# ReactiveBayes/RxInfer.jl

Hardware: AMD Instinct MI355X
Metric: node-message-updates/sec (d=4 LGSSM, T=100k, BP sweep with Bethe free energy) (higher is better)
Workload: dtype f64; 1 GPU; LGSSM d=4 dy=4 T=100000, 1024 independent chains per GPU (BASELINE config 2), 1 BP sweep + Bethe free energy per step; chain c drawn from numpy default_rng(42+c); chains_per_gpu=1024, T=100000, segments=128, segment_len=782

## Files before the change

### rxinfer.jl_amd/csrc/lgssm_kernels.hpp

```cpp
#pragma once
#include <hip/hip_runtime.h>
#include <stdint.h>

namespace rxhip {

constexpr int ST_NOT_POSDEF = 1;
constexpr int ST_NONFINITE = 2;
__device__ __forceinline__ void lds_barrier() {
    __builtin_amdgcn_fence(__ATOMIC_RELEASE, "workgroup", "local");
    __builtin_amdgcn_s_barrier();
    __builtin_amdgcn_fence(__ATOMIC_ACQUIRE, "workgroup", "local");
}
__device__ __forceinline__ bool is_finite(double x) { return (__double2hiint(x) & 0x7ff00000) != 0x7ff00000; }

#ifndef RXHIP_NT_STORES
#define RXHIP_NT_STORES 0
#endif
typedef double rx_d2v __attribute__((ext_vector_type(2)));
__device__ __forceinline__ void stream_store(double2* p, double a, double b) {
#if RXHIP_NT_STORES
    rx_d2v v = {a, b};
    __builtin_nontemporal_store(v, reinterpret_cast<rx_d2v*>(p));
#else
    *p = make_double2(a, b);
#endif
}

template <int D>
struct Dim {
    static constexpr int NS = D * (D + 1) / 2;
    static constexpr int NP = D + NS;
    static constexpr int NP2 = (NP + 1) / 2;
};

__host__ __device__ constexpr int sidx(int i, int j) { return i >= j ? i * (i + 1) / 2 + j : j * (j + 1) / 2 + i; }
// ... 965 lines not shown
    for (int q = 0; q < NS; ++q) {
        al[AL::J + q] = x[(EX::J + q) * p.n_chains];
        al[AL::C + q] = x[(EX::C + q) * p.n_chains];
    }
    if (!derived) return true;
    Sym<D> C, Ci;
    double det;
#pragma unroll
    for (int q = 0; q < NS; ++q) C.v[q] = al[AL::C + q];
    const bool ok = spd_inv<D>(C, Ci, det);
#pragma unroll
    for (int q = 0; q < NS; ++q) al[AL::CI + q] = Ci.v[q];
#pragma unroll
    for (int a = 0; a < D; ++a)
#pragma unroll
        for (int c = 0; c < D; ++c) {
            double acc = 0.0;
#pragma unroll
            for (int k = 0; k < D; ++k) acc += Ci(a, k) * al[AL::PI + k * D + c];
            al[AL::X + a * D + c] = acc;
        }
#pragma unroll
    for (int a = 0; a < D; ++a)
#pragma unroll
        for (int c = 0; c <= a; ++c) {
            double acc = al[AL::J + sidx(a, c)];
#pragma unroll
            for (int k = 0; k < D; ++k) acc += al[AL::PI + k * D + a] * al[AL::X + k * D + c];
            al[AL::JJ + sidx(a, c)] = acc;
        }
    return ok;
}

template <int D, int DY, bool FE, bool CK = false>
__global__ void __launch_bounds__(64) k_forward0(Params p, const CstArg<CstLayout<D, DY>::SIZE> cb) {
    using CL = CstLayout<D, DY>;
    using FL = F0Layout<D, DY>;
    constexpr int MT = TimeTab<D>::MT;
    constexpr int MP2 = DimM<D>::MP2;
    constexpr int U = 4;
    constexpr int NPF = U * FL::SIZE / 2;
    constexpr int NPM = U * MT / 2;
    constexpr int NPC = NPF + NPM;
    constexpr int PPL = (NPC + 63) / 64;
    __shared__ double2 tbuf[2][NPC];
    const int lane = threadIdx.x;
    const long long g = (long long)blockIdx.x * blockDim.x + threadIdx.x;
    const long long total = p.n_chains * (long long)p.S;
    const bool live = g < total;
    const long long seg = live ? g / p.n_chains : 0;
    const long long chain = live ? g - seg * p.n_chains : 0;
    const long long len = live ? seg_len(p, seg) : 0;
    const CPtr c{cb.v};
    const long long t0 = seg * p.L + 1;
    const long long seg0 = __builtin_amdgcn_readfirstlane((int)seg);
    const bool straddle = __builtin_amdgcn_ballot_w64(live && seg != seg0) != 0;
    const long long tw0 = seg0 * p.L + 1;
    const long long f_pieces = p.L * (FL::SIZE / 2);
    const long long m_pieces = p.T * (MT / 2);
    const double2* f2 = reinterpret_cast<const double2*>(p.ftab);
    const double2* m2 = reinterpret_cast<const double2*>(p.mtab);

    double2 tr[PPL];
    auto fetch = [&](long long i0) {
#pragma unroll
        for (int k = 0; k < PPL; ++k) {
// ... 2120 lines not shown
    constexpr int NS = Dim<D>::NS;
    {
        double mp[D], yv[DY];
        Sym<D> Vp, V;
#pragma unroll
        for (int i = 0; i < D; ++i) mp[i] = c[CL::M1 + i];
#pragma unroll
        for (int i = 0; i < NS; ++i) Vp.v[i] = c[CL::V1 + i];
        load_y<DY>(p.y, 0, p.n_chains, chain, yv);
        bool ok = true;
        double quad = 0.0, detprod = 1.0;
        obs_update<D, DY, true>(c, mp, Vp, yv, mseg, V, ok, quad, detprod);
        if (seg == 0) {
            store_filt_sh<D>(p, 0, chain, mseg, V);
            if (fe) p.fe_part[chain] = -0.5 * (quad + log(detprod));
            if (!ok) atomicOr(p.status, ST_NOT_POSDEF);
        }
    }
    boundary_chain<D, false>(p, chain - lane, (unsigned)lane, 0, (int)seg, lds, mseg);
#pragma unroll
    for (int i = 0; i < D; ++i) xb[i] = 0.0;
    boundary_chain<D, true>(p, chain - lane, (unsigned)lane, p.S - 1, p.S - 1 - (int)seg, lds, xb);
    const double* row = p.scan + seg * SL::SIZE;
    Sym<D> Vb, Lb;
#pragma unroll
    for (int i = 0; i < NS; ++i) {
        Vb.v[i] = row[SL::VB + i];
        Lb.v[i] = (seg == p.S - 1) ? 0.0 : row[SL::LB + i];
    }
    store_soa<D>(p.fstart, seg, p.n_chains, chain, mseg, Vb);
    store_soa<D>(p.beta, seg + 1, p.n_chains, chain, xb, Lb);
}

template <int D, int DY>
__global__ void __launch_bounds__(64) k_backward_sh_rev(Params p, const double* __restrict__ gtab, const double* __restrict__ segend,
                                                        const CstArg<CstLayout<D, DY>::SIZE> cb, const int bnd, const int write_cov) {
    using ST = SmoothTab<D>;
    using CL = CstLayout<D, DY>;
    constexpr int MP2 = DimM<D>::MP2;
    constexpr int MT = TimeTab<D>::MT;
    constexpr int U = 4;
    constexpr int RP = ST::SIZE / 2;
    constexpr int NPC = U * RP;
    constexpr int PPL = (NPC + 63) / 64;
    constexpr int NMP = 32 * D;
    constexpr int NCP = 32 * D * D;
    __shared__ double2 tbuf[2][NPC];
    __shared__ double mtile[64 * D];
    __shared__ double bndbuf[2][BndStage<D>::N];
    const int lane = threadIdx.x;
    const long long g0 = (long long)blockIdx.x * 64;
    const long long seg = g0 / p.n_chains;
    const long long chain0 = g0 - seg * p.n_chains;
    const long long chain = chain0 + lane;
    const long long len = seg_len(p, seg);
    const long long tb = seg * p.L, te = tb + len;
    const CPtr c{cb.v};
    const int lg = p.ck_log2;
    const long long K = 1LL << lg;
    auto load_ck = [&](long long t, double2 (&r)[MP2]) { load_filt_m_sh<D>(p, 1 + seg * p.nck + ((t - tb - 1) >> lg), chain, r); };
    double mseg[D];
    auto ck_mean = [&](const double2 (&r)[MP2], long long t, double (&mf)[D]) {
        unpack_m_sh<D>(r, mf);
        const double* N = p.ntab + t * MT;
#pragma unroll
        for (int i = 0; i < D; ++i) {
            double s = mf[i];
#pragma unroll
            for (int k = 0; k < D; ++k) s += N[i * D + k] * mseg[k];
            mf[i] = s;
        }
    };

    double mf[D], ms[D];
    {
        double xb[D];
        if (bnd) boundary_in_sweep<D, DY>(p, c, seg, chain, lane, bnd == 2, bndbuf, mseg, xb);
        else {
            const double* q = p.fstart + (seg * Dim<D>::NP) * p.n_chains + chain;
            const double* bq = p.beta + ((seg + 1) * Dim<D>::NP) * p.n_chains + chain;
#pragma unroll
            for (int i = 0; i < D; ++i) {
                mseg[i] = q[i * p.n_chains];
                xb[i] = bq[i * p.n_chains];
            }
        }
        if (len > 0) {
            double2 r[MP2];
            load_ck(te, r);
            ck_mean(r, te, mf);
        } else {
#pragma unroll
            for (int i = 0; i < D; ++i) mf[i] = mseg[i];
        }
        const double* se = segend + seg * SegEndTab<D>::SIZE;
#pragma unroll
        for (int i = 0; i < D; ++i) {
            double s = 0.0;
#pragma unroll
            for (int k = 0; k < D; ++k) s += se[SegEndTab<D>::H1 + i * D + k] * mf[k] + se[SegEndTab<D>::H2 + i * D + k] * xb[k];
            ms[i] = s;
        }
    }
    auto write_out = [&](long long t, const double* vs) {
#pragma unroll
        for (int i = 0; i < D; ++i) mtile[lane * D + i] = ms[i];
        __builtin_amdgcn_fence(__ATOMIC_RELEASE, "wavefront");
        __builtin_amdgcn_wave_barrier();
        __builtin_amdgcn_fence(__ATOMIC_ACQUIRE, "wavefront");
        double2* om = reinterpret_cast<double2*>(p.mean + (t * p.n_chains + chain0) * D);
        double2* oc = reinterpret_cast<double2*>(p.cov + (t * p.n_chains + chain0) * D * D);
#pragma unroll
        for (int k = 0; k < (NMP + 63) / 64; ++k) {
            const int q = k * 64 + lane;
            if (q < NMP) stream_store(om + q, mtile[2 * q], mtile[2 * q + 1]);
        }
        if (write_cov) {
#pragma unroll
            for (int k = 0; k < (NCP + 63) / 64; ++k) {
                const int q = k * 64 + lane;
                if (q < NCP) stream_store(oc + q, vs[(2 * q) % (D * D)], vs[(2 * q + 1) % (D * D)]);
            }
        }
        __builtin_amdgcn_fence(__ATOMIC_RELEASE, "wavefront");
        __builtin_amdgcn_wave_barrier();
    };
    if (seg == p.S - 1) write_out(te, gtab + te * ST::SIZE + ST::VS);

    const double2* g2 = reinterpret_cast<const double2*>(gtab);
    double2 tr[PPL];
    auto fetch = [&](long long i0) {
#pragma unroll
        for (int k = 0; k < PPL; ++k) {
            const int idx = k * 64 + lane;
            const long long r = i0 + idx / RP;
            tr[k] = (idx < NPC && r < len) ? g2[(te - 1 - r) * RP + idx % RP] : make_double2(0.0, 0.0);
        }
    };
    auto stash = [&](int b) {
#pragma unroll
        for (int k = 0; k < PPL; ++k) {
            const int idx = k * 64 + lane;
            if (idx < NPC) tbuf[b][idx] = tr[k];
        }
    };
    fetch(0);
    stash(0);
    __builtin_amdgcn_fence(__ATOMIC_RELEASE, "wavefront");
    __builtin_amdgcn_wave_barrier();
    long long tc = len > 0 ? tb + (((len - 1) >> lg) << lg) : tb;
    double2 rc[MP2];
    if (tc > tb) load_ck(tc, rc);
    double yn[DY];
    if (len > 0) load_y<DY>(p.y, te, p.n_chains, chain, yn);
    int b = 0;
    for (long long i0 = 0; i0 < len; i0 += U, b ^= 1) {
        if (i0 + U < len) fetch(i0 + U);
#pragma unroll
        for (int u = 0; u < U; ++u) {
            const long long i = i0 + u;
            if (i < len) {
                const long long t = te - 1 - i;
                const double* row = reinterpret_cast<const double*>(&tbuf[b][0]) + u * ST::SIZE;
                double yb[DY];
#pragma unroll
                for (int k = 0; k < DY; ++k) yb[k] = yn[k];
                if (t > tb) load_y<DY>(p.y, t, p.n_chains, chain, yn);
                double mfn[D];
                if (t == tb) {
#pragma unroll
                    for (int k = 0; k < D; ++k) mfn[k] = mseg[k];
                } else if (t == tc) {
                    ck_mean(rc, t, mfn);
                    tc -= K;
                    if (tc > tb) load_ck(tc, rc);
                } else {
                    double w[D], mp[D];
#pragma unroll
                    for (int a = 0; a < D; ++a) {
                        double s = 0.0;
#pragma unroll
                        for (int k = 0; k < D; ++k) s += c[CL::LOBS + sidx(a, k)] * mf[k];
#pragma unroll
                        for (int k = 0; k < DY; ++k) s -= c[CL::G + a * DY + k] * yb[k];
                        w[a] = s;
                    }
#pragma unroll
                    for (int a = 0; a < D; ++a) {
                        double s = mf[a];
#pragma unroll
                        for (int k = 0; k < D; ++k) s += row[ST::F + a * D + k] * w[k];
                        mp[a] = s;
                    }
#pragma unroll
                    for (int a = 0; a < D; ++a) {
                        double s = 0.0;
#pragma unroll
                        for (int k = 0; k < D; ++k) s += p.ainv[a * D + k] * mp[k];
                        mfn[a] = s;
                    }
                }
                double mn[D];
#pragma unroll
                for (int a = 0; a < D; ++a) {
                    double s0 = 0.0, s1 = 0.0;
#pragma unroll
                    for (int k = 0; k < D; ++k) {
                        s0 += row[ST::E + a * D + k] * mfn[k];
                        s1 += row[ST::G + a * D + k] * ms[k];
                    }
                    mn[a] = s0 + s1;
                }
#pragma unroll
                for (int a = 0; a < D; ++a) {
                    ms[a] = mn[a];
                    mf[a] = mfn[a];
                }
                write_out(t, row + ST::VS);
            }
        }
        __builtin_amdgcn_fence(__ATOMIC_ACQUIRE, "wavefront");
        __builtin_amdgcn_wave_barrier();
        if (i0 + U < len) stash(b ^ 1);
        __builtin_amdgcn_fence(__ATOMIC_RELEASE, "wavefront");
        __builtin_amdgcn_wave_barrier();
    }
}

}
```

### rxinfer.jl_amd/csrc/launch_tables.hpp

```cpp
#pragma once
#include <hip/hip_runtime.h>

#include <cstdlib>

#include "lgssm_kernels.hpp"
#include "predict_kernels.hpp"
#include "noise_kernels.hpp"
#ifndef RXHIP_LAUNCH_LGSSM_ONLY
#include "dense_kernels.hpp"
#include "dense_tab_kernels.hpp"
#include "dense_mseg_kernels.hpp"
#include "dense_split_kernels.hpp"
#include "dense8_kernels.hpp"
#endif

#ifndef RXHIP_TAB_SAME_TOL
#define RXHIP_TAB_SAME_TOL 5e-15
#endif

namespace rxhip {

struct LgssmVtbl {
    int d, dy;
    int cst_size, tab_size, agg_size;
    int oA, oP, oLOBS, oG, oQI, oC0, oM1, oV1, oHF;
    int tK, tU;
    int aPI, aC, aJ, aCI, aX, aJJ;
    int scan_size, sM1, sM2, sVB, sN1, sN2, sLB;
    int f0_size, fK, fU, fSI, pos_size, pPI, pJ, pC, fs_size, fsA1, fsA2, fsW, mt_row;
    void (*forward0)(const Params&, const double*, bool, bool, hipStream_t);
    void (*time_tables)(const TimeTabParams&, hipStream_t);
    void (*fe_seg)(const Params&, hipStream_t);
    int gt_row, se_size;
    void (*smooth_tables)(const SmoothTabParams&, const double*, hipStream_t);
    void (*backward_sh)(const Params&, const double*, const double*, const double*, bool, int, bool, hipStream_t);
    void (*boundary_scan_tab)(const Params&, const double*, bool, hipStream_t);
    void (*seg_aggregate)(const Params&, const double*, bool, hipStream_t);
    int ex_size;
    void (*seg_elements)(const Params&, hipStream_t);
    void (*boundary_scan)(const Params&, const double*, bool, bool, hipStream_t);
    void (*forward)(const Params&, const double*, bool, bool, hipStream_t);
    void (*backward)(const Params&, const double*, bool, hipStream_t);
    void (*forecast)(const PredictParams&, hipStream_t);
    void (*predict)(const PredictParams&, hipStream_t);
    void (*joint)(const PredictParams&, hipStream_t);
    void (*stream_step)(const StreamParams&, hipStream_t);
    void (*small_sweep)(const Params&, const double*, bool, hipStream_t);
    int noise_prior_size;
    void (*noise_reset)(const NoiseParams&, hipStream_t);
    void (*noise_update)(const NoiseParams&, hipStream_t);
};
void lgssm_vtbls_d1(LgssmVtbl* out);
void lgssm_vtbls_d2(LgssmVtbl* out);
void lgssm_vtbls_d3(LgssmVtbl* out);
void lgssm_vtbls_d4(LgssmVtbl* out);

inline unsigned nblk(long long n, int b) { return (unsigned)((n + b - 1) / b); }

inline const char* hook_env(const char* name) {
    const char* on = std::getenv("RXHIP_TEST_HOOKS");
    return (on && on[0] == '1' && on[1] == 0) ? std::getenv(name) : nullptr;
}

#ifndef RXHIP_LAUNCH_LGSSM_ONLY
constexpr int FE_RESID_MAX_PASSES = 8;
struct DenseVtbl {
    int nt;
    hipError_t (*prepare)();
// ... 26 lines not shown
```

### rxinfer.jl_amd/csrc/lgssm_plan.hpp

```cpp
#pragma once
#include <algorithm>
#include <cmath>
#include <cstdlib>
#include <cstring>
#include <string>

namespace rxhip {
namespace plan {

#define RXHIP_SCHEDULE_HOOKS(X)                                                                                                        \
    X(int, one_pass, -1)                                                                          \
    X(bool, one_segment, false)                                                                                  \
    X(bool, backward_lanes, false)                                                                            \
    X(bool, mean_records, false)                                                                              \
    X(int, mean_checkpoint, 0)                    \
    X(Text, mean_checkpoint_text, Text{})                                                   \
    X(bool, boundary_kernel, false)                                                                        \
    X(bool, small_sweep_off, false)                                                                            \
    X(bool, elem_full, false)                                                                                      \
    X(bool, noise_moments_pass, false)                                                                    \
    X(bool, no_pack, false)                                                                                          \
    X(int, dense_split, -1)                                      \
    X(bool, host_tables, false)                                                                                  \
    X(bool, gseq, false)                                                                                                \
    X(bool, stepm_gseq, false)                                                                                    \
    X(bool, filter_gseq, false)                                                                                  \
    X(bool, joints_gseq, false)                                                                                  \
    X(int, mseg_scan, 0)                                                 \
    X(bool, mseg_one_level, false)                                                                            \
    X(int, mseg_group, 0)                                                                          \
    X(unsigned long long, mseg_max_bytes, ~0ULL)                                         \
    X(bool, wave8_off, false)                                                                                        \
    X(bool, no_frozen, false)                                                                                      \
    X(bool, cov_every_sweep, false)

struct Text { char s[16] = {0}; };

struct ScheduleHooks {
#define X(type, field, dflt) type field = dflt;
    RXHIP_SCHEDULE_HOOKS(X)
#undef X
    template <class Get>
    static ScheduleHooks read(Get get) {
        ScheduleHooks h;
        auto set = [&](const char* n) { return get(n) != nullptr; };
        auto is0 = [&](const char* n) { const char* v = get(n); return v && std::atoi(v) == 0; };
        auto not0 = [&](const char* n) { const char* v = get(n); return v && std::atoi(v) != 0; };
        auto tri = [&](const char* n) { const char* v = get(n); return v ? (std::atoi(v) != 0 ? 1 : 0) : -1; };
        auto num = [&](const char* n) { const char* v = get(n); return v ? std::atoi(v) : 0; };
        h.one_pass = tri("RXHIP_ONE_PASS");
        h.one_segment = set("RXHIP_ONE_SEGMENT");
        h.backward_lanes = set("RXHIP_BACKWARD_LANES");
        h.mean_records = not0("RXHIP_MEAN_RECORDS");
        if (const char* v = get("RXHIP_MEAN_CHECKPOINT")) {
            h.mean_checkpoint = std::atoi(v);
            if (h.mean_checkpoint == 0) h.mean_checkpoint = -1;
            std::strncpy(h.mean_checkpoint_text.s, v, sizeof h.mean_checkpoint_text.s - 1);
        }
        h.boundary_kernel = not0("RXHIP_BOUNDARY_KERNEL");
        h.small_sweep_off = is0("RXHIP_SMALL_SWEEP");
        h.elem_full = set("RXHIP_ELEM_FULL");
        h.noise_moments_pass = set("RXHIP_NOISE_MOMENTS_PASS");
        h.no_pack = set("RXHIP_NO_PACK");
        h.dense_split = tri("RXHIP_DENSE_SPLIT");
        h.host_tables = set("RXHIP_HOST_TABLES");
        h.gseq = set("RXHIP_GSEQ");
        h.stepm_gseq = set("RXHIP_STEPM_GSEQ");
        h.filter_gseq = set("RXHIP_FILTER_GSEQ");
        h.joints_gseq = set("RXHIP_JOINTS_GSEQ");
        if (const char* v = get("RXHIP_MSEG_SCAN")) h.mseg_scan = !std::strcmp(v, "sequential") ? 1 : !std::strcmp(v, "log") ? 2 : 0;
        h.mseg_one_level = set("RXHIP_MSEG_ONE_LEVEL");
        h.mseg_group = num("RXHIP_MSEG_GROUP");
        if (const char* v = get("RXHIP_MSEG_MAX_BYTES")) h.mseg_max_bytes = std::strtoull(v, nullptr, 10);
        h.wave8_off = is0("RXHIP_WAVE8");
        h.no_frozen = set("RXHIP_NO_FROZEN");
        h.cov_every_sweep = not0("RXHIP_COV_EVERY_SWEEP");
        return h;
    }
    void append_key(std::string& key) const {
#define X(type, field, dflt) key.append(reinterpret_cast<const char*>(&field), sizeof field);
        RXHIP_SCHEDULE_HOOKS(X)
#undef X
    }
};

struct Shape {
    int d = 0, dy = 0;
    long long T = 0, n_chains = 0;
    int n_models = 1;
    long long segments = 0;
    bool dense = false, allow_missing = false, step_model = false, chain_model = false;
};

struct Flags {
    bool sequential = false, uniform = true, gseq = false, masked = false;
    int dpad = 0, nt = 0;
    int pack = 1;
    long long wg_chains = 0;
    int dyk = 0;
};
inline Flags static_flags(const Shape& s, const ScheduleHooks& hooks) {
    Flags f;
    f.dpad = s.dense ? (s.d + 15) / 16 * 16 : s.d;
    f.nt = f.dpad / 16;
    f.uniform = (s.n_models == 1);
    if (s.allow_missing) {
        if (s.dense) f.gseq = true;
        f.masked = true;
        f.sequential = true;
// ... 70 lines not shown
```

### rxinfer.jl_amd/csrc/rxhip.hip

```cpp
#include "../../include/rxhip.h"

#include <hip/hip_runtime.h>

#include <algorithm>
#include <cmath>
#include <mutex>
#include <set>
#include <cstdarg>
#include <cstdio>
#include <cstring>
#include <cstdlib>
#include <string>
#include <vector>

#include "launch_tables.hpp"
#include "gseq_kernels.hpp"
#include "drift_kernels.hpp"
#include "generic_kernels.hpp"
#include "engine.hpp"
#include "graph_lowering.hpp"
#include "model_envelope.hpp"

using namespace rxhip;
using plan::ScheduleHooks;
// ... 1942 lines not shown
    std::vector<double> cst((size_t)e->n_models * vt->cst_size), tab((size_t)e->n_models * Ltab * vt->tab_size + 1),
        agg((size_t)e->n_models * 2 * vt->agg_size), scan;
    FusedTables ft;
    const bool want_fused = plan::want_fused(e->uniform, e->S, e->n_chains, e->T, e->hooks);
    StageTrace tr(e->stage_ms);
    for (int m = 0; m < e->n_models; ++m) {
        rxhip_status st = build_model_tables(e, m, ds, cst.data() + (size_t)m * vt->cst_size,
                                             tab.data() + (size_t)m * Ltab * vt->tab_size,
                                             agg.data() + (size_t)m * 2 * vt->agg_size, e->uniform ? &scan : nullptr,
                                             want_fused ? &ft : nullptr);
        if (st) return st;
    }
    e->fused = want_fused && !scan.empty();
    e->fe_const = ft.fe_const;
    e->h_cst0.assign(cst.begin(), cst.begin() + vt->cst_size);
    tr.mark("lanes: host tables", STAGE_TABLES_HOST);
    const size_t C = (size_t)e->n_chains, T = (size_t)e->T, Sg = (size_t)(e->S > 0 ? e->S : 1);
    ArenaPlan ap;
    ap.upload(&e->d_cst, cst.data(), sizeof(double) * cst.size());
    ap.upload(&e->d_tab, tab.data(), sizeof(double) * tab.size());
    ap.upload(&e->d_agg, agg.data(), sizeof(double) * agg.size());
    if (ds->chain_model && !e->uniform) ap.upload(&e->d_chain_model, ds->chain_model, sizeof(int) * C);
    if (ds->step_model) ap.upload(&e->d_step_model, ds->step_model, sizeof(int) * (size_t)(e->T + e->H));
    if (!e->h_mu.empty()) {
        ap.upload(&e->d_mu, e->h_mu.data(), sizeof(double) * e->h_mu.size());
        ap.upload(&e->d_nu, e->h_nu.data(), sizeof(double) * e->h_nu.size());
        ap.upload(&e->d_cx, e->h_cx.data(), sizeof(double) * e->h_cx.size());
        ap.upload(&e->d_cy_raw, e->h_cy.data(), sizeof(double) * e->h_cy.size());
    }
    if (e->uniform && !scan.empty()) ap.upload(&e->d_scan, scan.data(), sizeof(double) * scan.size());
    const int ck_forced = e->hooks.mean_checkpoint;
    if (ck_forced && (ck_forced < 1 || ck_forced > 32 || (ck_forced & (ck_forced - 1))))
        return fail(e, RXHIP_ERR_BADARG, "RXHIP_MEAN_CHECKPOINT=%s: a power of two from 1 to 32", e->hooks.mean_checkpoint_text.s);
    const bool rev_cand = plan::rev_cand(e->fused, e->n_chains, e->d, e->dy, e->T, e->hooks);
    if (e->fused) {
        ap.upload(&e->d_ftab, ft.ftab.data(), sizeof(double) * ft.ftab.size());
        ap.upload(&e->d_pos, ft.pos.data(), sizeof(double) * ft.pos.size());
        ap.upload(&e->d_fseg, ft.fseg.data(), sizeof(double) * ft.fseg.size());
        ap.plain(&e->d_mtab, sizeof(double) * T * vt->mt_row);
        ap.plain(&e->d_ntab, sizeof(double) * T * vt->mt_row);
        if (plan::gtab_tables(e->n_chains, e->hooks)) {
            ap.plain(&e->d_gtab, sizeof(double) * T * vt->gt_row);
            ap.plain(&e->d_segend, sizeof(double) * Sg * vt->se_size);
            ap.plain(&e->d_sblk, sizeof(double) * Sg * (size_t)smooth_blocks_per_segment(e->L) * 3 * e->d * e->d);
        }
        if (rev_cand) {
            ap.plain(&e->d_amp, sizeof(double) * T);
            ap.zeroed(&e->d_ainv, sizeof(double) * e->d * e->d);
            ap.zeroed(&e->d_ckfail, sizeof(int));
        }
    }
    ap.zeroed_last(&e->d_status, sizeof(int));
    ap.zeroed(&e->d_fe_part, sizeof(double) * (Sg + 2) * C);
    e->fe_total_cap = 16;
    ap.zeroed(&e->d_fe_total, sizeof(double) * e->fe_total_cap);
    ap.plain(&e->d_fe_blocks, sizeof(double) * ((C + 63) / 64));
    if (e->uniform) {
        const size_t MP2 = ((size_t)e->d + 1) / 2;
        if (!rev_cand) ap.plain(&e->d_filt, sizeof(double) * T * MP2 * 2 * (((C + 63) / 64) * 64));
        ap.plain(&e->d_vtab, sizeof(double) * T * ((size_t)e->d * (e->d + 1) / 2));
    } else
        ap.plain(&e->d_filt, sizeof(double) * T * NP2 * 2 * (((C + 63) / 64) * 64));
    ap.plain_first(&e->d_mean, sizeof(double) * (size_t)e->Tout() * C * e->d);
    ap.plain_first(&e->d_cov, sizeof(double) * (size_t)e->Tout() * C * e->d * e->d);
    ap.plain_first(&e->d_fe_chain, sizeof(double) * C);
    ap.plain(&e->d_elem, sizeof(double) * Sg * 2 * e->d * C);
// ... 627 lines not shown
    rxhip_status st;
    const bool fe = pl.fe, fused = pl.family == RunFamily::OnePass, bnd_in_sweep = pl.bnd_in_sweep;
    if (fused) {
        if ((st = prof_begin(e, RXHIP_K_FORWARD))) return st;
        e->vt->forward0(p, e->h_cst0.data(), fe, e->ck_log2 > 0, e->stream);
        if ((st = prof_end(e))) return st;
    } else if (pl.family == RunFamily::SmallSweep) {
        e->vt->small_sweep(p, e->h_cst0.data(), fe, e->stream);
        return RXHIP_OK;
    } else if (pl.family == RunFamily::FourPhase) {
        if ((st = prof_begin(e, RXHIP_K_SEG_AGGREGATE))) return st;
        e->vt->seg_aggregate(p, e->h_cst0.data(), e->uniform, e->stream);
        if ((st = prof_end(e))) return st;
    } else if (pl.elements_pass) {
        if ((st = prof_begin(e, RXHIP_K_SEG_AGGREGATE))) return st;
        e->vt->seg_elements(p, e->stream);
        if ((st = prof_end(e))) return st;
    }
    if (!bnd_in_sweep) {
        if ((st = prof_begin(e, RXHIP_K_BOUNDARY_SCAN))) return st;
        if (pl.scan_tab) e->vt->boundary_scan_tab(p, e->h_cst0.data(), fe, e->stream);
        else e->vt->boundary_scan(p, e->h_cst0.data(), e->uniform, fe, e->stream);
        if ((st = prof_end(e))) return st;
    }
    if (pl.segments) {
        if (!fused) {
            if ((st = prof_begin(e, RXHIP_K_FORWARD))) return st;
            e->vt->forward(p, e->h_cst0.data(), e->uniform, fe, e->stream);
            if ((st = prof_end(e))) return st;
        } else if (fe && !bnd_in_sweep)
            e->vt->fe_seg(p, e->stream);
        if (!pl.filter) {
            if ((st = prof_begin(e, RXHIP_K_BACKWARD))) return st;
            if (pl.backward_sh) e->vt->backward_sh(p, e->h_cst0.data(), e->d_gtab, e->d_segend, e->ck_log2 > 0, bnd_in_sweep ? (fe ? 2 : 1) : 0, write_cov, e->stream);
            else e->vt->backward(p, e->h_cst0.data(), e->uniform, e->stream);
            if ((st = prof_end(e))) return st;
        }
        if (fe && bnd_in_sweep) e->vt->fe_seg(p, e->stream);
    }
    return RXHIP_OK;
}
static rxhip_status run_tail(rxhip_engine* e, const RunPlan& pl, const Params& p, const DenseParams& dp, NoiseParams& np, int it) {
    rxhip_status st;
    if (e->noise) {
        np.iteration = it;
        e->vt->noise_update(np, e->stream);
    }
    if (pl.fe && pl.family != RunFamily::SmallSweep) {
        if ((st = prof_begin(e, RXHIP_K_FE_REDUCE))) return st;
        const int nb = (int)((e->n_chains + 63) / 64);
        Params pr = p;
        pr.S = pl.fe_slots;
        pr.fe_part = pl.fe_part;
        if (pl.info && (pl.family == RunFamily::Dense || pl.family == RunFamily::DenseSplit)) launch_fe_resid(dp, e->stream);
        if (e->n_chains <= 16) {
            hipLaunchKernelGGL(k_fe_few, dim3(1), dim3(256), 0, e->stream, pr);
        } else {
            hipLaunchKernelGGL(k_fe_chain, dim3(nb), dim3(256), 0, e->stream, pr, e->d_fe_blocks);
            hipLaunchKernelGGL(k_fe_total, dim3(1), dim3(256), 0, e->stream, p, (const double*)e->d_fe_blocks, nb);
        }
        if ((st = prof_end(e))) return st;
    }
    if (e->d_mu) {
        hipLaunchKernelGGL(k_shift_rows, dim3(2048), dim3(256), 0, e->stream, e->d_mean, (const double*)e->d_mu, e->T, e->n_chains, e->d, 1.0, e->off_chain ? 1 : 0);
    }
    if (e->H > 0 && e->dense) {
        GenericParams gp{};
// ... 578 lines not shown
```

### rxinfer.jl_amd/csrc/tu_lgssm.hip

```cpp
#include <cstring>

#define RXHIP_LAUNCH_LGSSM_ONLY
#include "launch_tables.hpp"

#ifndef RXHIP_TU_D
#error "compile with -DRXHIP_TU_D=1..4"
#endif

namespace rxhip {
namespace {

template <int D, int DY>
struct Launch {
    using CL = CstLayout<D, DY>;
    static CstArg<CL::SIZE> carg(const double* hc) {
        CstArg<CL::SIZE> a;
        std::memcpy(a.v, hc, sizeof(double) * CL::SIZE);
        return a;
    }
    static void seg_aggregate(const Params& p, const double* hc, bool uni, hipStream_t s) {
        const long long total = p.n_chains * (long long)p.S;
        if (uni) hipLaunchKernelGGL((k_seg_aggregate<D, DY, true>), dim3(nblk(total, 64)), dim3(64), 0, s, p, carg(hc));
    }
    static void seg_elements(const Params& p, hipStream_t s) {
// ... 40 lines not shown
        else forward_t<false>(p, hc, uni, fe, s);
    }
    static void backward(const Params& p, const double* hc, bool uni, hipStream_t s) {
        const long long total = p.n_chains * (long long)p.S;
        dim3 grid(nblk(total, 64));
        if (uni && p.ntab) hipLaunchKernelGGL((k_backward<D, DY, true, true>), grid, dim3(64), 0, s, p, carg(hc));
        else if (uni) hipLaunchKernelGGL((k_backward<D, DY, true>), grid, dim3(64), 0, s, p, carg(hc));
        else if (p.noise_part && p.tinv_records) hipLaunchKernelGGL((k_backward_noise<D, DY, true>), grid, dim3(64), 0, s, p);
        else if (p.noise_part) hipLaunchKernelGGL((k_backward_noise<D, DY>), grid, dim3(64), 0, s, p);
        else if (p.tinv_records) hipLaunchKernelGGL((k_backward_tinv<D, DY>), grid, dim3(64), 0, s, p);
        else hipLaunchKernelGGL((k_backward<D, DY, false>), grid, dim3(64), 0, s, p, CstArg<1>{});
    }
    static void forward0(const Params& p, const double* hc, bool fe, bool ck, hipStream_t s) {
        const long long total = p.n_chains * (long long)p.S;
        if (ck) {
            if (fe) hipLaunchKernelGGL((k_forward0<D, DY, true, true>), dim3(nblk(total, 64)), dim3(64), 0, s, p, carg(hc));
            else hipLaunchKernelGGL((k_forward0<D, DY, false, true>), dim3(nblk(total, 64)), dim3(64), 0, s, p, carg(hc));
        } else if (fe) hipLaunchKernelGGL((k_forward0<D, DY, true>), dim3(nblk(total, 64)), dim3(64), 0, s, p, carg(hc));
        else hipLaunchKernelGGL((k_forward0<D, DY, false>), dim3(nblk(total, 64)), dim3(64), 0, s, p, carg(hc));
    }
    static void time_tables(const TimeTabParams& q, hipStream_t s) {
        hipLaunchKernelGGL((k_time_tables<D>), dim3(nblk(q.T, 64)), dim3(64), 0, s, q);
    }
    static void fe_seg(const Params& p, hipStream_t s) {
        hipLaunchKernelGGL((k_fe_seg<D>), dim3(nblk(p.n_chains * (long long)p.S, 64)), dim3(64), 0, s, p);
    }
    static void smooth_tables(const SmoothTabParams& q, const double* hc, hipStream_t s) {
        const long long nblocks = (long long)q.S * smooth_blocks_per_segment(q.L);
        if (q.T > 1) hipLaunchKernelGGL((k_smooth_tab_steps<D, DY>), dim3(nblk(q.T - 1, 64)), dim3(64), 0, s, q, carg(hc));
        hipLaunchKernelGGL((k_smooth_tab_compose<D>), dim3(nblk(nblocks, 64)), dim3(64), 0, s, q);
        hipLaunchKernelGGL((k_smooth_tab_chain<D>), dim3(nblk(q.S, 64)), dim3(64), 0, s, q);
        hipLaunchKernelGGL((k_smooth_tab_apply<D>), dim3(nblk(nblocks, 64)), dim3(64), 0, s, q);
    }
    static void backward_sh(const Params& p, const double* hc, const double* gtab, const double* segend, bool rev, int bnd, bool write_cov, hipStream_t s) {
        if (rev) hipLaunchKernelGGL((k_backward_sh_rev<D, DY>), dim3((unsigned)(p.n_chains / 64 * p.S)), dim3(64), 0, s, p, gtab, segend, carg(hc), bnd, write_cov ? 1 : 0);
        else hipLaunchKernelGGL((k_backward_sh<D>), dim3((unsigned)(p.n_chains / 64 * p.S)), dim3(64), 0, s, p, gtab, segend, write_cov ? 1 : 0);
    }
    static void forecast(const PredictParams& p, hipStream_t s) {
        hipLaunchKernelGGL((k_forecast<D, DY>), dim3(nblk(p.n_chains, 64)), dim3(64), 0, s, p);
    }
    static void predict(const PredictParams& p, hipStream_t s) {
        const long long total = (p.T + p.H) * p.n_chains;
        const long long nb = (total + 255) / 256;
        hipLaunchKernelGGL((k_predict<D, DY>), dim3((unsigned)(nb < 8192 ? nb : 8192)), dim3(256), 0, s, p);
    }
    static void joint(const PredictParams& p, hipStream_t s) {
        const long long nb = ((p.T - 1) * p.n_chains + 255) / 256;
        hipLaunchKernelGGL((k_joint<D, DY>), dim3((unsigned)(nb < 8192 ? (nb > 0 ? nb : 1) : 8192)), dim3(256), 0, s, p);
    }
    static void small_sweep(const Params& p, const double* hc, bool fe, hipStream_t s) {
        const size_t lds = sizeof(double) * (size_t)small_sweep_lds_doubles<D, DY>();
        const int par = p.S >= 24 ? 1 : 0;
        if (p.filter) {
            if (fe) hipLaunchKernelGGL((k_small_sweep<D, DY, true, true>), dim3(1), dim3(SMALL_SWEEP_THREADS), lds, s, p, carg(hc), par);
            else hipLaunchKernelGGL((k_small_sweep<D, DY, false, true>), dim3(1), dim3(SMALL_SWEEP_THREADS), lds, s, p, carg(hc), par);
        } else if (fe) hipLaunchKernelGGL((k_small_sweep<D, DY, true, false>), dim3(1), dim3(SMALL_SWEEP_THREADS), lds, s, p, carg(hc), par);
        else hipLaunchKernelGGL((k_small_sweep<D, DY, false, false>), dim3(1), dim3(SMALL_SWEEP_THREADS), lds, s, p, carg(hc), par);
    }
    static void noise_reset(const NoiseParams& p, hipStream_t s) {
        hipLaunchKernelGGL((k_noise_reset<D, DY>), dim3(nblk(p.n_chains, 64)), dim3(64), 0, s, p);
    }
    static void noise_update(const NoiseParams& p, hipStream_t s) {
        if (!p.moments_in_sweep) hipLaunchKernelGGL((k_noise_moments<D, DY>), dim3(nblk(p.n_chains, 64), (unsigned)p.slices), dim3(64), 0, s, p);
        hipLaunchKernelGGL((k_noise_update<D, DY>), dim3(nblk(p.n_chains, 64)), dim3(64), 0, s, p);
    }
    static void stream_step(const StreamParams& p, hipStream_t s) {
        hipLaunchKernelGGL((k_stream_step<D, DY>), dim3(nblk(p.n_chains, 64)), dim3(64), 0, s, p);
    }
// ... 56 lines not shown
```

Measured before the change: 245.3 billion rule-calls/s.

## Prefetch observations and checkpoints a chunk ahead in backward smoother via ring buffer

Restructures the backward smoothing loop so observations and checkpoint filtered means for the next chunk are loaded into a register ring one chunk ahead, instead of being loaded per step just before use. It also stages the Ainv matrix and checkpoint N-row in shared memory, and makes table fetches branch-free by clamping indices. Full chunks run through an unrolled ring with compile-time-resolved bounds checks. The intent is to hide global load latency on the serial recurrence, at the cost of more registers and extra wave barriers in ck_mean.

```diff
diff --git a/rxinfer.jl_amd/csrc/lgssm_kernels.hpp b/rxinfer.jl_amd/csrc/lgssm_kernels.hpp
--- a/rxinfer.jl_amd/csrc/lgssm_kernels.hpp
+++ b/rxinfer.jl_amd/csrc/lgssm_kernels.hpp
@@ -1,6 +1,7 @@
 #pragma once
 #include <hip/hip_runtime.h>
 #include <stdint.h>
+#include <type_traits>
 
 namespace rxhip {
 
@@ -1032,6 +1033,12 @@
     return ok;
 }
 
+#ifndef RXHIP_Y_AHEAD
+#define RXHIP_Y_AHEAD 1
+#endif
+constexpr int Y_AHEAD_BWD = RXHIP_Y_AHEAD;
+static_assert(Y_AHEAD_BWD >= 1, "the ring holds the chunk in use and at least one ahead");
+
 template <int D, int DY, bool FE, bool CK = false>
 __global__ void __launch_bounds__(64) k_forward0(Params p, const CstArg<CstLayout<D, DY>::SIZE> cb) {
     using CL = CstLayout<D, DY>;
@@ -3234,6 +3241,8 @@
     __shared__ double2 tbuf[2][NPC];
     __shared__ double mtile[64 * D];
     __shared__ double bndbuf[2][BndStage<D>::N];
+    __shared__ double ainv_s[D * D];
+    __shared__ double nrow_s[MT];
     const int lane = threadIdx.x;
     const long long g0 = (long long)blockIdx.x * 64;
     const long long seg = g0 / p.n_chains;
@@ -3244,11 +3253,18 @@
     const CPtr c{cb.v};
     const int lg = p.ck_log2;
     const long long K = 1LL << lg;
-    auto load_ck = [&](long long t, double2 (&r)[MP2]) { load_filt_m_sh<D>(p, 1 + seg * p.nck + ((t - tb - 1) >> lg), chain, r); };
+    auto load_ck = [&](long long t, double2 (&r)[MP2], double& n) {
+        load_filt_m_sh<D>(p, 1 + seg * p.nck + ((t - tb - 1) >> lg), chain, r);
+        n = p.ntab[t * MT + (lane < MT ? lane : 0)];
+    };
     double mseg[D];
-    auto ck_mean = [&](const double2 (&r)[MP2], long long t, double (&mf)[D]) {
+    auto ck_mean = [&](const double2 (&r)[MP2], const double n, double (&mf)[D]) {
         unpack_m_sh<D>(r, mf);
-        const double* N = p.ntab + t * MT;
+        if (lane < MT) nrow_s[lane] = n;
+        __builtin_amdgcn_fence(__ATOMIC_RELEASE, "wavefront");
+        __builtin_amdgcn_wave_barrier();
+        __builtin_amdgcn_fence(__ATOMIC_ACQUIRE, "wavefront");
+        const double* N = nrow_s;
 #pragma unroll
         for (int i = 0; i < D; ++i) {
             double s = mf[i];
@@ -3256,6 +3272,8 @@
             for (int k = 0; k < D; ++k) s += N[i * D + k] * mseg[k];
             mf[i] = s;
         }
+        __builtin_amdgcn_fence(__ATOMIC_RELEASE, "wavefront");
+        __builtin_amdgcn_wave_barrier();
     };
 
     double mf[D], ms[D];
@@ -3273,8 +3291,9 @@
         }
         if (len > 0) {
             double2 r[MP2];
-            load_ck(te, r);
-            ck_mean(r, te, mf);
+            double n;
+            load_ck(te, r, n);
+            ck_mean(r, n, mf);
         } else {
 #pragma unroll
             for (int i = 0; i < D; ++i) mf[i] = mseg[i];
@@ -3314,52 +3333,81 @@
     if (seg == p.S - 1) write_out(te, gtab + te * ST::SIZE + ST::VS);
 
     const double2* g2 = reinterpret_cast<const double2*>(gtab);
-    double2 tr[PPL];
-    auto fetch = [&](long long i0) {
+    auto fetch = [&](long long i0, rx_d2v (&tr)[PPL]) {
+#pragma unroll
+        for (int k = 0; k < PPL; ++k) {
+            const int idx = k * 64 + lane < NPC ? k * 64 + lane : NPC - 1;
+            const long long r = te - 1 - (i0 + idx / RP);
+            tr[k] = *reinterpret_cast<const rx_d2v*>(g2 + (r > tb ? r : tb) * RP + idx % RP);
+        }
+    };
+    auto stash = [&](int b, const rx_d2v (&tr)[PPL]) {
 #pragma unroll
         for (int k = 0; k < PPL; ++k) {
             const int idx = k * 64 + lane;
-            const long long r = i0 + idx / RP;
-            tr[k] = (idx < NPC && r < len) ? g2[(te - 1 - r) * RP + idx % RP] : make_double2(0.0, 0.0);
+            if (idx < NPC) *reinterpret_cast<rx_d2v*>(&tbuf[b][idx]) = tr[k];
         }
     };
-    auto stash = [&](int b) {
-#pragma unroll
-        for (int k = 0; k < PPL; ++k) {
-            const int idx = k * 64 + lane;
-            if (idx < NPC) tbuf[b][idx] = tr[k];
-        }
-    };
-    fetch(0);
-    stash(0);
+    {
+        rx_d2v tr[PPL];
+        fetch(0, tr);
+        stash(0, tr);
+    }
+    if (lane < D * D) ainv_s[lane] = p.ainv[lane];
     __builtin_amdgcn_fence(__ATOMIC_RELEASE, "wavefront");
     __builtin_amdgcn_wave_barrier();
-    long long tc = len > 0 ? tb + (((len - 1) >> lg) << lg) : tb;
-    double2 rc[MP2];
-    if (tc > tb) load_ck(tc, rc);
-    double yn[DY];
-    if (len > 0) load_y<DY>(p.y, te, p.n_chains, chain, yn);
+    constexpr int AH = Y_AHEAD_BWD, NR = AH + 1;
+    constexpr int LGU = 2;
+    static_assert(U == 1 << LGU, "a chunk holds at most one checkpoint when K >= U");
+    double yr[NR][U][DY];
+    double2 rcr[NR][MP2];
+    double ncr[NR];
+    auto load_chunk_ck = [&](long long c0, double2 (&r)[MP2], double& n) {
+        const long long tck = tb + (((te - 1 - c0 - tb) >> lg) << lg);
+        load_ck(tck > tb ? tck : te, r, n);
+    };
+    const double* const ylo = p.y + (tb * p.n_chains + chain) * DY;
+    const double* ynext = p.y + (te * p.n_chains + chain) * DY;
+    const long long ystr = p.n_chains * DY;
+    auto load_chunk_y = [&](double (&ys)[U][DY]) {
+#pragma unroll
+        for (int u = 0; u < U; ++u) {
+            load_y<DY>(ynext, 0, 0, 0, ys[u]);
+            ynext = ynext - ylo >= ystr ? ynext - ystr : ylo;
+        }
+    };
+#pragma unroll
+    for (int a = 0; a < AH; ++a) {
+        load_chunk_y(yr[a]);
+        load_chunk_ck(a * U, rcr[a], ncr[a]);
+    }
     int b = 0;
-    for (long long i0 = 0; i0 < len; i0 += U, b ^= 1) {
-        if (i0 + U < len) fetch(i0 + U);
+    auto chunk = [&](const long long i0, const int sc, const int sa, auto full) {
+        constexpr bool FULL = decltype(full)::value;
+        const double (&yc)[U][DY] = yr[sc];
+        rx_d2v tr[PPL];
+        fetch(i0 + U, tr);
+        load_chunk_y(yr[sa]);
+        load_chunk_ck(i0 + AH * U, rcr[sa], ncr[sa]);
 #pragma unroll
         for (int u = 0; u < U; ++u) {
             const long long i = i0 + u;
-            if (i < len) {
+            if (FULL || i < len) {
                 const long long t = te - 1 - i;
                 const double* row = reinterpret_cast<const double*>(&tbuf[b][0]) + u * ST::SIZE;
-                double yb[DY];
-#pragma unroll
-                for (int k = 0; k < DY; ++k) yb[k] = yn[k];
-                if (t > tb) load_y<DY>(p.y, t, p.n_chains, chain, yn);
+                const double (&yb)[DY] = yc[u];
                 double mfn[D];
                 if (t == tb) {
 #pragma unroll
                     for (int k = 0; k < D; ++k) mfn[k] = mseg[k];
-                } else if (t == tc) {
-                    ck_mean(rc, t, mfn);
-                    tc -= K;
-                    if (tc > tb) load_ck(tc, rc);
+                } else if (((t - tb) & (K - 1)) == 0) {
+                    if (lg >= LGU) ck_mean(rcr[sc], ncr[sc], mfn);
+                    else {
+                        double2 r[MP2];
+                        double n;
+                        load_ck(t, r, n);
+                        ck_mean(r, n, mfn);
+                    }
                 } else {
                     double w[D], mp[D];
 #pragma unroll
@@ -3382,7 +3430,7 @@
                     for (int a = 0; a < D; ++a) {
                         double s = 0.0;
 #pragma unroll
-                        for (int k = 0; k < D; ++k) s += p.ainv[a * D + k] * mp[k];
+                        for (int k = 0; k < D; ++k) s += ainv_s[a * D + k] * mp[k];
                         mfn[a] = s;
                     }
                 }
@@ -3407,10 +3455,19 @@
         }
         __builtin_amdgcn_fence(__ATOMIC_ACQUIRE, "wavefront");
         __builtin_amdgcn_wave_barrier();
-        if (i0 + U < len) stash(b ^ 1);
+        stash(b ^ 1, tr);
         __builtin_amdgcn_fence(__ATOMIC_RELEASE, "wavefront");
         __builtin_amdgcn_wave_barrier();
-    }
-}
-
-}
+        b ^= 1;
+    };
+    long long i0 = 0;
+    for (; i0 + NR * U <= len; i0 += NR * U) {
+#pragma unroll
+        for (int r = 0; r < NR; ++r) chunk(i0 + r * U, r, (r + AH) % NR, std::true_type{});
+    }
+#pragma unroll
+    for (int r = 0; r < NR; ++r)
+        if (i0 + r * U < len) chunk(i0 + r * U, r, (r + AH) % NR, std::false_type{});
+}
+
+}
```

After: 236.1 billion rule-calls/s. 0.963x the previous value.

## Deepen y prefetch ring and restructure reverse-filter backward sweep loop

Applied to the files above, without the earlier changes.

The reverse-filter smoothing kernel now keeps a compile-time ring of R observation vectors (default 4) loaded several steps ahead, instead of one step ahead. Checkpoint means and their N-table row are prefetched early and staged through LDS. The A-inverse matrix is cached in LDS rather than read from global memory. The main loop is split into a full-block body with no bounds checks plus a tail, with clamped fetches and compile-time-known store guards. This is meant to hide global load latency in the serial per-step recurrence, at the cost of more registers for the ring, which may lower occupancy.

```diff
diff --git a/rxinfer.jl_amd/csrc/launch_tables.hpp b/rxinfer.jl_amd/csrc/launch_tables.hpp
--- a/rxinfer.jl_amd/csrc/launch_tables.hpp
+++ b/rxinfer.jl_amd/csrc/launch_tables.hpp
@@ -33,7 +33,7 @@
     void (*fe_seg)(const Params&, hipStream_t);
     int gt_row, se_size;
     void (*smooth_tables)(const SmoothTabParams&, const double*, hipStream_t);
-    void (*backward_sh)(const Params&, const double*, const double*, const double*, bool, int, bool, hipStream_t);
+    void (*backward_sh)(const Params&, const double*, const double*, const double*, bool, int, bool, int, hipStream_t);
     void (*boundary_scan_tab)(const Params&, const double*, bool, hipStream_t);
     void (*seg_aggregate)(const Params&, const double*, bool, hipStream_t);
     int ex_size;
diff --git a/rxinfer.jl_amd/csrc/lgssm_kernels.hpp b/rxinfer.jl_amd/csrc/lgssm_kernels.hpp
--- a/rxinfer.jl_amd/csrc/lgssm_kernels.hpp
+++ b/rxinfer.jl_amd/csrc/lgssm_kernels.hpp
@@ -3218,7 +3218,11 @@
     store_soa<D>(p.beta, seg + 1, p.n_chains, chain, xb, Lb);
 }
 
-template <int D, int DY>
+#ifndef RXHIP_Y_RING_DEPTH
+#define RXHIP_Y_RING_DEPTH 4
+#endif
+constexpr int Y_RING_SHIPPED = RXHIP_Y_RING_DEPTH;
+template <int D, int DY, int R>
 __global__ void __launch_bounds__(64) k_backward_sh_rev(Params p, const double* __restrict__ gtab, const double* __restrict__ segend,
                                                         const CstArg<CstLayout<D, DY>::SIZE> cb, const int bnd, const int write_cov) {
     using ST = SmoothTab<D>;
@@ -3231,9 +3235,13 @@
     constexpr int PPL = (NPC + 63) / 64;
     constexpr int NMP = 32 * D;
     constexpr int NCP = 32 * D * D;
+    static_assert(U % R == 0, "ring slots must be compile-time");
+    static_assert(MT <= 64, "one lane per element of an N row");
     __shared__ double2 tbuf[2][NPC];
     __shared__ double mtile[64 * D];
     __shared__ double bndbuf[2][BndStage<D>::N];
+    __shared__ double ainv[D * D];
+    __shared__ double nrow[MT];
     const int lane = threadIdx.x;
     const long long g0 = (long long)blockIdx.x * 64;
     const long long seg = g0 / p.n_chains;
@@ -3246,9 +3254,8 @@
     const long long K = 1LL << lg;
     auto load_ck = [&](long long t, double2 (&r)[MP2]) { load_filt_m_sh<D>(p, 1 + seg * p.nck + ((t - tb - 1) >> lg), chain, r); };
     double mseg[D];
-    auto ck_mean = [&](const double2 (&r)[MP2], long long t, double (&mf)[D]) {
+    auto ck_mean = [&](const double2 (&r)[MP2], const double* N, double (&mf)[D]) {
         unpack_m_sh<D>(r, mf);
-        const double* N = p.ntab + t * MT;
 #pragma unroll
         for (int i = 0; i < D; ++i) {
             double s = mf[i];
@@ -3274,7 +3281,7 @@
         if (len > 0) {
             double2 r[MP2];
             load_ck(te, r);
-            ck_mean(r, te, mf);
+            ck_mean(r, p.ntab + te * MT, mf);
         } else {
 #pragma unroll
             for (int i = 0; i < D; ++i) mf[i] = mseg[i];
@@ -3299,118 +3306,136 @@
 #pragma unroll
         for (int k = 0; k < (NMP + 63) / 64; ++k) {
             const int q = k * 64 + lane;
-            if (q < NMP) stream_store(om + q, mtile[2 * q], mtile[2 * q + 1]);
+            if ((k + 1) * 64 <= NMP || q < NMP) stream_store(om + q, mtile[2 * q], mtile[2 * q + 1]);
         }
         if (write_cov) {
 #pragma unroll
             for (int k = 0; k < (NCP + 63) / 64; ++k) {
                 const int q = k * 64 + lane;
-                if (q < NCP) stream_store(oc + q, vs[(2 * q) % (D * D)], vs[(2 * q + 1) % (D * D)]);
+                if ((k + 1) * 64 <= NCP || q < NCP) stream_store(oc + q, vs[(2 * q) % (D * D)], vs[(2 * q + 1) % (D * D)]);
             }
         }
         __builtin_amdgcn_fence(__ATOMIC_RELEASE, "wavefront");
         __builtin_amdgcn_wave_barrier();
     };
     if (seg == p.S - 1) write_out(te, gtab + te * ST::SIZE + ST::VS);
-
-    const double2* g2 = reinterpret_cast<const double2*>(gtab);
-    double2 tr[PPL];
+    if (len <= 0) return;
+
+    const rx_d2v* g2 = reinterpret_cast<const rx_d2v*>(gtab);
+    rx_d2v tr[PPL];
     auto fetch = [&](long long i0) {
+#pragma unroll
+        for (int k = 0; k < PPL; ++k) {
+            const int idx = k * 64 + lane < NPC ? k * 64 + lane : NPC - 1;
+            const long long r = i0 + idx / RP;
+            tr[k] = g2[(te - 1 - (r < len ? r : len - 1)) * RP + idx % RP];
+        }
+    };
+    auto stash = [&](int b) {
 #pragma unroll
         for (int k = 0; k < PPL; ++k) {
             const int idx = k * 64 + lane;
-            const long long r = i0 + idx / RP;
-            tr[k] = (idx < NPC && r < len) ? g2[(te - 1 - r) * RP + idx % RP] : make_double2(0.0, 0.0);
-        }
-    };
-    auto stash = [&](int b) {
-#pragma unroll
-        for (int k = 0; k < PPL; ++k) {
-            const int idx = k * 64 + lane;
-            if (idx < NPC) tbuf[b][idx] = tr[k];
+            if ((k + 1) * 64 <= NPC || idx < NPC) tbuf[b][idx] = make_double2(tr[k].x, tr[k].y);
         }
     };
     fetch(0);
+    if (lane < D * D) ainv[lane] = p.ainv[lane];
     stash(0);
     __builtin_amdgcn_fence(__ATOMIC_RELEASE, "wavefront");
     __builtin_amdgcn_wave_barrier();
-    long long tc = len > 0 ? tb + (((len - 1) >> lg) << lg) : tb;
+    long long tc = tb + (((len - 1) >> lg) << lg);
     double2 rc[MP2];
-    if (tc > tb) load_ck(tc, rc);
-    double yn[DY];
-    if (len > 0) load_y<DY>(p.y, te, p.n_chains, chain, yn);
+    double nc;
+    auto prefetch_ck = [&]() {
+        const long long t = tc > tb ? tc : (tb + K < te ? tb + K : te);
+        load_ck(t, rc);
+        nc = p.ntab[t * MT + (lane < MT ? lane : MT - 1)];
+    };
+    prefetch_ck();
+    double yr[R][DY];
+    auto y_index = [&](long long i) { return te - (i < len ? i : len - 1); };
+#pragma unroll
+    for (int r = 0; r < R; ++r) load_y<DY>(p.y, y_index(r), p.n_chains, chain, yr[r]);
+    auto step = [&](const int u, const long long i, const int b) __attribute__((always_inline)) {
+        const long long t = te - 1 - i;
+        const double* row = reinterpret_cast<const double*>(&tbuf[b][0]) + u * ST::SIZE;
+        const double (&yb)[DY] = yr[u % R];
+        double mfn[D];
+        if (t == tb) {
+#pragma unroll
+            for (int k = 0; k < D; ++k) mfn[k] = mseg[k];
+        } else if (t == tc) {
+            if (lane < MT) nrow[lane] = nc;
+            __builtin_amdgcn_fence(__ATOMIC_RELEASE, "wavefront");
+            __builtin_amdgcn_wave_barrier();
+            __builtin_amdgcn_fence(__ATOMIC_ACQUIRE, "wavefront");
+            ck_mean(rc, nrow, mfn);
+            __builtin_amdgcn_fence(__ATOMIC_RELEASE, "wavefront");
+            __builtin_amdgcn_wave_barrier();
+            __builtin_amdgcn_sched_barrier(0);
+            tc -= K;
+            prefetch_ck();
+        } else {
+            double w[D], mp[D];
+#pragma unroll
+            for (int a = 0; a < D; ++a) {
+                double s = 0.0;
+#pragma unroll
+                for (int k = 0; k < D; ++k) s += c[CL::LOBS + sidx(a, k)] * mf[k];
+#pragma unroll
+                for (int k = 0; k < DY; ++k) s -= c[CL::G + a * DY + k] * yb[k];
+                w[a] = s;
+            }
+#pragma unroll
+            for (int a = 0; a < D; ++a) {
+                double s = mf[a];
+#pragma unroll
+                for (int k = 0; k < D; ++k) s += row[ST::F + a * D + k] * w[k];
+                mp[a] = s;
+            }
+#pragma unroll
+            for (int a = 0; a < D; ++a) {
+                double s = 0.0;
+#pragma unroll
+                for (int k = 0; k < D; ++k) s += ainv[a * D + k] * mp[k];
+                mfn[a] = s;
+            }
+        }
+        __builtin_amdgcn_sched_barrier(0);
+        load_y<DY>(p.y, y_index(i + R), p.n_chains, chain, yr[u % R]);
+        double mn[D];
+#pragma unroll
+        for (int a = 0; a < D; ++a) {
+            double s0 = 0.0, s1 = 0.0;
+#pragma unroll
+            for (int k = 0; k < D; ++k) {
+                s0 += row[ST::E + a * D + k] * mfn[k];
+                s1 += row[ST::G + a * D + k] * ms[k];
+            }
+            mn[a] = s0 + s1;
+        }
+#pragma unroll
+        for (int a = 0; a < D; ++a) {
+            ms[a] = mn[a];
+            mf[a] = mfn[a];
+        }
+        write_out(t, row + ST::VS);
+    };
     int b = 0;
-    for (long long i0 = 0; i0 < len; i0 += U, b ^= 1) {
-        if (i0 + U < len) fetch(i0 + U);
-#pragma unroll
-        for (int u = 0; u < U; ++u) {
-            const long long i = i0 + u;
-            if (i < len) {
-                const long long t = te - 1 - i;
-                const double* row = reinterpret_cast<const double*>(&tbuf[b][0]) + u * ST::SIZE;
-                double yb[DY];
-#pragma unroll
-                for (int k = 0; k < DY; ++k) yb[k] = yn[k];
-                if (t > tb) load_y<DY>(p.y, t, p.n_chains, chain, yn);
-                double mfn[D];
-                if (t == tb) {
-#pragma unroll
-                    for (int k = 0; k < D; ++k) mfn[k] = mseg[k];
-                } else if (t == tc) {
-                    ck_mean(rc, t, mfn);
-                    tc -= K;
-                    if (tc > tb) load_ck(tc, rc);
-                } else {
-                    double w[D], mp[D];
-#pragma unroll
-                    for (int a = 0; a < D; ++a) {
-                        double s = 0.0;
-#pragma unroll
-                        for (int k = 0; k < D; ++k) s += c[CL::LOBS + sidx(a, k)] * mf[k];
-#pragma unroll
-                        for (int k = 0; k < DY; ++k) s -= c[CL::G + a * DY + k] * yb[k];
-                        w[a] = s;
-                    }
-#pragma unroll
-                    for (int a = 0; a < D; ++a) {
-                        double s = mf[a];
-#pragma unroll
-                        for (int k = 0; k < D; ++k) s += row[ST::F + a * D + k] * w[k];
-                        mp[a] = s;
-                    }
-#pragma unroll
-                    for (int a = 0; a < D; ++a) {
-                        double s = 0.0;
-#pragma unroll
-                        for (int k = 0; k < D; ++k) s += p.ainv[a * D + k] * mp[k];
-                        mfn[a] = s;
-                    }
-                }
-                double mn[D];
-#pragma unroll
-                for (int a = 0; a < D; ++a) {
-                    double s0 = 0.0, s1 = 0.0;
-#pragma unroll
-                    for (int k = 0; k < D; ++k) {
-                        s0 += row[ST::E + a * D + k] * mfn[k];
-                        s1 += row[ST::G + a * D + k] * ms[k];
-                    }
-                    mn[a] = s0 + s1;
-                }
-#pragma unroll
-                for (int a = 0; a < D; ++a) {
-                    ms[a] = mn[a];
-                    mf[a] = mfn[a];
-                }
-                write_out(t, row + ST::VS);
-            }
-        }
+    long long i0 = 0;
+    for (; i0 + U <= len; i0 += U, b ^= 1) {
+        fetch(i0 + U);
+#pragma unroll
+        for (int u = 0; u < U; ++u) step(u, i0 + u, b);
         __builtin_amdgcn_fence(__ATOMIC_ACQUIRE, "wavefront");
         __builtin_amdgcn_wave_barrier();
-        if (i0 + U < len) stash(b ^ 1);
+        stash(b ^ 1);
         __builtin_amdgcn_fence(__ATOMIC_RELEASE, "wavefront");
         __builtin_amdgcn_wave_barrier();
     }
-}
-
-}
+#pragma unroll
+    for (int u = 0; u < U - 1; ++u)
+        if (i0 + u < len) step(u, i0 + u, b);
+}
+
+}
diff --git a/rxinfer.jl_amd/csrc/lgssm_plan.hpp b/rxinfer.jl_amd/csrc/lgssm_plan.hpp
--- a/rxinfer.jl_amd/csrc/lgssm_plan.hpp
+++ b/rxinfer.jl_amd/csrc/lgssm_plan.hpp
@@ -32,7 +32,8 @@
     X(unsigned long long, mseg_max_bytes, ~0ULL)                                         \
     X(bool, wave8_off, false)                                                                                        \
     X(bool, no_frozen, false)                                                                                      \
-    X(bool, cov_every_sweep, false)
+    X(bool, cov_every_sweep, false)                                                                        \
+    X(int, y_ring, 0)
 
 struct Text { char s[16] = {0}; };
 
@@ -75,6 +76,7 @@
         h.wave8_off = is0("RXHIP_WAVE8");
         h.no_frozen = set("RXHIP_NO_FROZEN");
         h.cov_every_sweep = not0("RXHIP_COV_EVERY_SWEEP");
+        if (const char* v = get("RXHIP_Y_RING")) h.y_ring = !std::strcmp(v, "1") ? 1 : -1;
         return h;
     }
     void append_key(std::string& key) const {
diff --git a/rxinfer.jl_amd/csrc/rxhip.hip b/rxinfer.jl_amd/csrc/rxhip.hip
--- a/rxinfer.jl_amd/csrc/rxhip.hip
+++ b/rxinfer.jl_amd/csrc/rxhip.hip
@@ -1998,6 +1998,8 @@
     const int ck_forced = e->hooks.mean_checkpoint;
     if (ck_forced && (ck_forced < 1 || ck_forced > 32 || (ck_forced & (ck_forced - 1))))
         return fail(e, RXHIP_ERR_BADARG, "RXHIP_MEAN_CHECKPOINT=%s: a power of two from 1 to 32", e->hooks.mean_checkpoint_text.s);
+    if (e->hooks.y_ring != 0 && e->hooks.y_ring != 1)
+        return fail(e, RXHIP_ERR_BADARG, "RXHIP_Y_RING: 1 (the depth-1 y ring of the reverse-filter sweep) or unset (depth %d)", Y_RING_SHIPPED);
     const bool rev_cand = plan::rev_cand(e->fused, e->n_chains, e->d, e->dy, e->T, e->hooks);
     if (e->fused) {
         ap.upload(&e->d_ftab, ft.ftab.data(), sizeof(double) * ft.ftab.size());
@@ -2691,7 +2693,7 @@
             e->vt->fe_seg(p, e->stream);
         if (!pl.filter) {
             if ((st = prof_begin(e, RXHIP_K_BACKWARD))) return st;
-            if (pl.backward_sh) e->vt->backward_sh(p, e->h_cst0.data(), e->d_gtab, e->d_segend, e->ck_log2 > 0, bnd_in_sweep ? (fe ? 2 : 1) : 0, write_cov, e->stream);
+            if (pl.backward_sh) e->vt->backward_sh(p, e->h_cst0.data(), e->d_gtab, e->d_segend, e->ck_log2 > 0, bnd_in_sweep ? (fe ? 2 : 1) : 0, write_cov, e->hooks.y_ring == 1 ? 1 : Y_RING_SHIPPED, e->stream);
             else e->vt->backward(p, e->h_cst0.data(), e->uniform, e->stream);
             if ((st = prof_end(e))) return st;
         }
diff --git a/rxinfer.jl_amd/csrc/tu_lgssm.hip b/rxinfer.jl_amd/csrc/tu_lgssm.hip
--- a/rxinfer.jl_amd/csrc/tu_lgssm.hip
+++ b/rxinfer.jl_amd/csrc/tu_lgssm.hip
@@ -96,8 +96,10 @@
         hipLaunchKernelGGL((k_smooth_tab_chain<D>), dim3(nblk(q.S, 64)), dim3(64), 0, s, q);
         hipLaunchKernelGGL((k_smooth_tab_apply<D>), dim3(nblk(nblocks, 64)), dim3(64), 0, s, q);
     }
-    static void backward_sh(const Params& p, const double* hc, const double* gtab, const double* segend, bool rev, int bnd, bool write_cov, hipStream_t s) {
-        if (rev) hipLaunchKernelGGL((k_backward_sh_rev<D, DY>), dim3((unsigned)(p.n_chains / 64 * p.S)), dim3(64), 0, s, p, gtab, segend, carg(hc), bnd, write_cov ? 1 : 0);
+    static void backward_sh(const Params& p, const double* hc, const double* gtab, const double* segend, bool rev, int bnd, bool write_cov, int y_ring, hipStream_t s) {
+        const dim3 grid((unsigned)(p.n_chains / 64 * p.S));
+        if (rev && y_ring == 1) hipLaunchKernelGGL((k_backward_sh_rev<D, DY, 1>), grid, dim3(64), 0, s, p, gtab, segend, carg(hc), bnd, write_cov ? 1 : 0);
+        else if (rev) hipLaunchKernelGGL((k_backward_sh_rev<D, DY, Y_RING_SHIPPED>), grid, dim3(64), 0, s, p, gtab, segend, carg(hc), bnd, write_cov ? 1 : 0);
         else hipLaunchKernelGGL((k_backward_sh<D>), dim3((unsigned)(p.n_chains / 64 * p.S)), dim3(64), 0, s, p, gtab, segend, write_cov ? 1 : 0);
     }
     static void forecast(const PredictParams& p, hipStream_t s) {
```

After: 258.0 billion rule-calls/s before, 289.8 billion rule-calls/s after, median of 6. 12.3% higher.
